# Unrepentant-Atheist/AC-3-ACM-Codec

Hardware: AMD Instinct MI355X
Metric: AC-3 5.1@48kHz frames/sec/GPU (decode+encode); achieved HBM GB/s vs peak (higher is better)
Workload: dtype f32+i32

## Files before the change

ac-3-acm-codec_amd/csrc/decode_mx.hip:

```cpp
#include <stdlib.h>
#include "mant2.h"
#include "xform_core.h"
#include "ac3mi_internal.h"

namespace ac3mi {

constexpr int MX_PLANE = 256 + 16;
constexpr int MX_WAVE = 6 * EX_GROUP * 8;
constexpr int MX_RING = 6 * MX_PLANE * 4;
constexpr int MX_TILE = 3072;
static_assert(MX_RING + M2_LDS_WAVE <= MX_WAVE && MX_TILE + 256 * 6 * 2 <= MX_WAVE && 48 * 8 * 8 <= MX_TILE, "region layout");

struct MantxParams {
    MantParams m;
    const uint8_t *blksw;
    float *delay;
    const int32_t *slot;
    int delay_stride;
    float *pcm;
    int16_t *pcm16;
    int8_t wslot[6];
    const float2 *tw_long, *tw_short;
    const float *window;
    float bias;
// ... 51 lines not shown
    const uint64_t rve = failed ? 0ull : D.rv_exp();
    const uint64_t rvb = failed ? 0ull : D.rv_bap();
    const uint8_t *const rowbase = P.rows + (size_t)fidx * 6 * ROWSET;
    const RowFetch fetch{rowbase, rve, rvb, lane};
    __builtin_assume(B.nf >= 1);
    const int slot0 = seg_slot(0, B.nf, B.chincpl, B.chincpl ? __builtin_ctz(B.chincpl) : 99);
    const uint2 first = fetch(slot0);
    {
        stage_frame_store<384>(frw, fw, P.frame_bytes, tid);
        if (const int own = D.own_bytes()) trim_staged_frame(frw, own, nw, tid, 384);
        if (tid < M2_NDESC) L.dsc[tid] = mant_desc2((uint32_t)tid);
        L.qtab[tid] = q0;
        if (tid < 760 - 384) L.qtab[384 + tid] = q1;
        reinterpret_cast<float2 *>(&L.tw[0][0])[tid] = twv;
        if (tid < 6) L.ready[tid] = 0u;
    }
    __syncthreads();
    MX_LAP(0);

    if (failed) {
        for (int c = 0; c < n_in; c++)
            *reinterpret_cast<float4 *>(planes + c * MX_PLANE + 4 * lane) = make_float4(0.f, 0.f, 0.f, 0.f);
    } else {
        D.ranges(B);
        B.gainv = D.gainv(lane);
        if (B.chincpl && lane < 18) {
            const uint32_t below = D.cplbndstrc() & ((1u << lane) - 1u);
            L.cplbnd[blk][lane] = (uint8_t)(lane - __popc(below));
        }
        const uint32_t fpos = rfl(fposv);
        const bool lfsr_live = fpos != 0xffffffffu;
        const uint32_t i0 = lfsr_live ? (fpos + D.draw_off()) % 65535u : 0u;
        const float *cc = P.cplco + unit * 90;
        mant_block2<MX_PLANE, true>(B, fetch, first, [&](int c, int bnd) { return cc[c * 18 + bnd]; }, L.cplbnd[blk], L.dsc, region + MX_RING, frw,
                              (uint32_t)nw + 2u, L.qtab, reinterpret_cast<const int16_t *>(P.lfsr_seq) + 1 + i0, lfsr_live, planes, D.bitpos(), lane);
    }
    wave_sync();

    MX_LAP(1);
    const int l8 = lane & 7, grp = lane >> 3;
    const bool own = grp < n_in;
    const int o = own ? grp : 0;
    const int fb = o - B.in_lfe;
    const bool sw = fb >= 0 && Q.blksw[unit * nfchans + fb] != 0;
    const size_t sidx = Q.slot ? (size_t)Q.slot[fidx] : (size_t)fidx;
    float *const dptr = Q.delay + sidx * Q.delay_stride + (size_t)o * 128;
    float2 dl[8];
    if (blk == 0) {
#pragma unroll
        for (int j = 0; j < 8; j++) {
            const int i = ((j & 1) ? 15 - l8 : l8) + 16 * (j >> 1);
            dl[j] = *reinterpret_cast<const float2 *>(dptr + 2 * i);
        }
    }
    FirstTail ft;
#pragma unroll
    for (int j = 0; j < 8; j++) ft.f0[j] = ft.f1[j] = ft.t0[j] = ft.t1[j] = 0.f;
    {
        const float *plane = planes + o * MX_PLANE;
        float xa[16], xb[16];
        if (!sw) {
            const float2 *p = reinterpret_cast<const float2 *>(plane) + l8;
            float2 v[16];
#pragma unroll
            for (int n = 0; n < 16; n++) v[n] = p[8 * n];
#pragma unroll
            for (int n = 0; n < 16; n++) {
// ... 31 lines not shown
    if (blk > 0) {
        for (int spin = 0; spin < (1 << 20) && __hip_atomic_load(&L.ready[blk - 1], __ATOMIC_ACQUIRE, __HIP_MEMORY_SCOPE_WORKGROUP) == 0u; spin++)
            __builtin_amdgcn_s_sleep(1);
        const float2 *tl = reinterpret_cast<const float2 *>(L.wave[blk - 1]);
        const int ls = lane < 48 ? lane : l8;
#pragma unroll
        for (int j = 0; j < 8; j++) dl[j] = tl[j * 48 + ls];
    }
    if (blk == 5) {
        for (int spin = 0; spin < (1 << 20) && __hip_atomic_load(&L.ready[0], __ATOMIC_ACQUIRE, __HIP_MEMORY_SCOPE_WORKGROUP) == 0u; spin++)
            __builtin_amdgcn_s_sleep(1);
    }
    if (blk == 5 && own) {
#pragma unroll
        for (int j = 0; j < 8; j++) {
            const int i = ((j & 1) ? 15 - l8 : l8) + 16 * (j >> 1);
            *reinterpret_cast<float2 *>(dptr + 2 * i) = make_float2(ft.t0[j], ft.t1[j]);
        }
    }

    MX_LAP(3);
    int16_t *tile = reinterpret_cast<int16_t *>(region + MX_TILE);
    int wsl = 0;
    if constexpr (FX) {
        uint64_t w = 0;
#pragma unroll
        for (int oo = 0; oo < 6; oo++) w |= (uint64_t)(uint8_t)Q.wslot[oo] << (8 * oo);
        wsl = (int)((uint32_t)(w >> (8 * o)) & 0xffu);
    } else {
#pragma unroll
        for (int oo = 0; oo < 6; oo++) wsl = oo == o ? Q.wslot[oo] : wsl;
    }
    float *oblk = S16 ? nullptr : Q.pcm + (unit * n_in + o) * 256;
#pragma unroll
    for (int j = 0; j < 8; j++) {
        const int i = ((j & 1) ? 15 - l8 : l8) + 16 * (j >> 1);
        const float2 wlo = *reinterpret_cast<const float2 *>(&L.win[2 * i]);
        const float2 whi = *reinterpret_cast<const float2 *>(&L.win[254 - 2 * i]);
        float2 lo, hi;
        window_pair(ft.f0[j], ft.f1[j], dl[j], wlo, whi, Q.bias, lo, hi);
        if (!S16 && own) {
            *reinterpret_cast<float2 *>(oblk + 2 * i) = lo;
            *reinterpret_cast<float2 *>(oblk + 254 - 2 * i) = hi;
        }
        if (S16 && own) {
            const int at = wsl + (int)__umul24((uint32_t)(2 * i), (uint32_t)n_in), top = wsl + (int)__umul24(254u, (uint32_t)n_in) - (at - wsl);
            tile[at] = to_s16(lo.x);
            tile[at + n_in] = to_s16(lo.y);
            tile[top] = to_s16(hi.x);
            tile[top + n_in] = to_s16(hi.y);
        }
    }
    if (S16) {
        wave_sync();
        const int upb = 32 * n_in;
        int16_t *dst = Q.pcm16 + unit * 256 * n_in;
#pragma unroll
        for (int it = 0; it < 3; it++) {
            const int u = it * 64 + lane;
            if (u < upb) *reinterpret_cast<uint4 *>(dst + u * 8) = *reinterpret_cast<const uint4 *>(tile + u * 8);
        }
    }
    MX_LAP(4);
}

template <uint32_t V> struct MantxVariant { static constexpr auto fn = mantx_kernel<(V & V_S16) != 0, (V & V_FX) != 0>; };

hipError_t launch_mantx(const DeviceTables &tab, const DecodeLaunch &L, const MantParams &M, const KernelLaunch &k, hipStream_t stream)
{
    if (!L.fuse) return hipErrorInvalidValue;
    const XformLaunch &X = *L.fuse;
    if (L.frames_per_stream != 1 || X.plan.n_in != X.plan.n_out || M.n_in > 6) return hipErrorInvalidValue;
    MantxParams Q;
    Q.m = M;
    Q.m.coef = nullptr;
    Q.blksw = L.blksw;
    Q.delay = X.delay;
    Q.slot = X.slot;
    Q.delay_stride = X.slot ? X.delay_stride : X.plan.n_out * 128;
// ... 32 lines not shown
```

ac-3-acm-codec_amd/csrc/mant2.h:

```cpp
#pragma once
#include "decode_common.h"

namespace ac3mi {

constexpr int M2_RING = 3 * 128;
constexpr int M2_LDS_WAVE = M2_RING + 256;
constexpr int M2_NDESC = 97;
constexpr int LFSR_EXT = 16384;


struct alignas(16) BlkDesc {
    uint32_t bitpos;
    uint32_t draw_off;
    uint32_t flags;
    uint32_t cplbndstrc;
    uint16_t endmant[5], cplstrt, cplend;
    uint16_t own_bytes;
    uint8_t rv_exp[8], rv_bap[8];
    float gain[5], lfe_gain;
    uint32_t src_snr;
    uint32_t pad1;
};
constexpr uint32_t BLK_FAILED = 1u;
constexpr int BLK_CHINCPL = 8, BLK_DITH = 16, BLK_REMAT = 24;
static_assert(sizeof(BlkDesc) == BLKDESC_BYTES && offsetof(BlkDesc, src_snr) == BLKDESC_SRC_SNR, "what the host sizes and reads (ac3mi_internal.h)");

constexpr int ROWSET = 7 * 512;

static_assert(offsetof(BlkDesc, bitpos) == 0 && offsetof(BlkDesc, draw_off) == 4 && offsetof(BlkDesc, flags) == 8 && offsetof(BlkDesc, cplbndstrc) == 12,
              "lanes 0-3: the first four dwords");
static_assert(offsetof(BlkDesc, cplstrt) == offsetof(BlkDesc, endmant) + 2 * 5 && offsetof(BlkDesc, cplend) == offsetof(BlkDesc, endmant) + 2 * 6 &&
              offsetof(BlkDesc, own_bytes) == offsetof(BlkDesc, endmant) + 2 * 7, "lanes 0-7: eight halfwords from endmant on; 6 = the coupling slot");
static_assert(offsetof(BlkDesc, lfe_gain) == offsetof(BlkDesc, gain) + 4 * 5 && offsetof(BlkDesc, src_snr) == offsetof(BlkDesc, gain) + 4 * 6,
              "lanes 0-6: seven dwords from gain on");
// ... 20 lines not shown
        return (flags & BLK_FAILED) != 0u;
    }
    __device__ __forceinline__ void ranges(MantBlk &B) const
    {
        constexpr size_t E = offsetof(BlkDesc, endmant);
        B.cplstrtmant = (int)s16<offsetof(BlkDesc, cplstrt)>(); B.cplendmant = (int)s16<offsetof(BlkDesc, cplend)>();
        B.ends = (uint64_t)((s16<E>() & 0xffu) | ((s16<E + 2>() & 0xffu) << 8) | ((s16<E + 4>() & 0xffu) << 16) | ((s16<E + 6>() & 0xffu) << 24)) |
                 ((uint64_t)(s16<E + 8>() & 0xffu) << 32);
    }
    __device__ __forceinline__ float gainv(int lane) const
    {
        constexpr size_t G = offsetof(BlkDesc, gain);
        return __uint_as_float(lane == 0 ? u32<G>() : lane == 1 ? u32<G + 4>() : lane == 2 ? u32<G + 8>() : lane == 3 ? u32<G + 12>()
                             : lane == 4 ? u32<G + 16>() : u32<offsetof(BlkDesc, lfe_gain)>());
    }
    __device__ __forceinline__ int own_bytes() const { return (int)s16<offsetof(BlkDesc, own_bytes)>(); }
    __device__ __forceinline__ uint32_t cplbndstrc() const { return s32<offsetof(BlkDesc, cplbndstrc)>(); }
    __device__ __forceinline__ uint32_t bitpos() const { return s32<offsetof(BlkDesc, bitpos)>(); }
    __device__ __forceinline__ uint32_t draw_off() const { return s32<offsetof(BlkDesc, draw_off)>(); }
    __device__ __forceinline__ uint64_t rv_exp() const { return (uint64_t)s32<offsetof(BlkDesc, rv_exp)>() | ((uint64_t)s32<offsetof(BlkDesc, rv_exp) + 4>() << 32); }
    __device__ __forceinline__ uint64_t rv_bap() const { return (uint64_t)s32<offsetof(BlkDesc, rv_bap)>() | ((uint64_t)s32<offsetof(BlkDesc, rv_bap) + 4>() << 32); }
};

struct RowFetch {
    const uint8_t *const &rowbase;
    const uint64_t &rve, &rvb;
    const int &lane;
    __device__ __forceinline__ uint2 operator()(int slot) const
    {
        const uint8_t *er = rowbase + (size_t)((rve >> (8 * slot)) & 7u) * ROWSET + slot * 512;
        const uint8_t *br = rowbase + (size_t)((rvb >> (8 * slot)) & 7u) * ROWSET + slot * 512 + 256;
        if (slot == 5) return lane < 7 ? make_uint2(br[lane], er[lane]) : make_uint2(1u, 0u);
        return make_uint2(reinterpret_cast<const uint32_t *>(br)[lane], reinterpret_cast<const uint32_t *>(er)[lane]);
    }
};

__host__ __device__ inline uint4 mant_desc2(uint32_t b)
{
    const uint32_t k1 = b >> 5, nbp = b >= 32 ? 0u : b == 1 ? 0u : b;
    const uint32_t inc = k1 == 1 ? 1u << 20 : k1 == 2 ? 1u << 10 : k1 == 3 ? 1u : 0u;
    const uint32_t obits = k1 == 1 ? 5u : k1 ? 7u : 0u, per = k1 == 3 ? 2u : k1 ? 3u : 0u, sh = 30u - 10u * k1;
    const uint32_t recip = k1 == 3 ? 1024u : k1 ? 683u : 0u;
    const uint32_t qbase = k1 == 1 ? 0u : k1 == 2 ? 96u : k1 == 3 ? 480u : nbp == 3 ? 736u : nbp == 4 ? 744u : 0u;
    const uint32_t coded = (k1 || nbp == 3 || nbp == 4) ? 1u : 0u, zero = b == 0 ? 1u : 0u;
    const uint32_t ring = k1 ? 128u * (k1 - 1u) : 0u;
    return make_uint4(inc, nbp | (obits << 8) | (per << 16) | (sh << 24), recip | (qbase << 16), ring | (zero << 16) | (coded << 24));
}

struct MantParams {
    const uint8_t *frames;
    const BlkDesc *desc;
    const uint8_t *rows;
    const float *cplco;
    const uint32_t *frame_pos;
    float *coef;
    const uint16_t *lfsr_seq;
    const DecTables *tab;
    unsigned n_frames;
    int frame_stride, frame_bytes;
    int acmod, lfeon, n_in, nfchans;
};

struct Seg2 {
    uint32_t bit;
    uint32_t phase;
    uint32_t draw;
// ... 24 lines not shown
    uint32_t nb[NB], nbsum = 0, ndsum = 0, slot[NB];
#pragma unroll
    for (int j = 0; j < NB; j++) {
        const uint32_t x = __builtin_amdgcn_ubfe(run, R.dy[j] >> 24, 10);
        run += inc[j];
        const uint32_t q = (x * (R.dz[j] & 0xffffu)) >> 11;
        const uint32_t mem = x - q * ((R.dy[j] >> 16) & 0xffu);
        const uint32_t ob = mem == 0u ? (R.dy[j] >> 8) & 0xffu : 0u;
        nb[j] = (R.dy[j] & 0xffu) + ob;
        nbsum += nb[j];
        ndsum += ((R.dw[j] >> 16) & 0xffu) * (uint32_t)mult;
        const uint32_t rslot = (R.dw[j] & 0xffffu) + (q & 127u);
        R.rs[j] = rslot | (mem << 16);
        slot[j] = ob != 0u ? rslot : (uint32_t)(M2_RING + 4 * lane);
    }
    const uint32_t bl = nbsum | (ndsum << 16);
    const uint32_t bin_ = wave_incl_scan_u32(bl);
    const uint32_t gtot = wave_last(gin), btot = wave_last(bin_);
    R.cd = S.draw + (bin_ >> 16) - ndsum;
    const uint32_t off = S.bit + (bin_ & 0xffffu) - nbsum;
    uint32_t wi = off >> 5;
    wi = wi < frw_last ? wi : frw_last;
    const uint32_t d0 = frw[wi], d1 = frw[wi + 1], d2 = frw[wi + 2];
    const uint32_t k = off & 31u;
    uint64_t win = ((((uint64_t)d0 << 32) | d1) << k) | (uint64_t)((d2 >> 1) >> (31u - k));
#pragma unroll
    for (int j = 0; j < NB; j++) {
        R.raw[j] = ((uint32_t)(win >> 32) >> 1) >> (31u - nb[j]);
        win <<= nb[j];
        ring[slot[j]] = (uint8_t)R.raw[j];
    }
    S.bit += btot & 0xffffu;
    S.draw += btot >> 16;
    {
        const uint32_t x3 = ((S.phase >> 20) & 1023u) + ((gtot >> 20) & 1023u), x5 = ((S.phase >> 10) & 1023u) + ((gtot >> 10) & 1023u),
                       x11 = (S.phase & 1023u) + (gtot & 1023u);
        const uint32_t q3 = (x3 * 683u) >> 11, q5 = (x5 * 683u) >> 11, q11 = x11 >> 1;
        S.phase = (((q3 & 127u) * 3u + (x3 - 3u * q3)) << 20) | (((q5 & 127u) * 3u + (x5 - 3u * q5)) << 10) | ((q11 & 127u) * 2u + (x11 & 1u));
    }
}

template <int NB>
__device__ __forceinline__ void seg2_values(const Bins2<NB> &R, const uint8_t *ring, const float *qtab, float *q)
{
    uint32_t code[NB];
#pragma unroll
    for (int j = 0; j < NB; j++) code[j] = ring[R.rs[j] & 0xffffu];
#pragma unroll
    for (int j = 0; j < NB; j++) { asm volatile("" : "+v"(code[j])); code[j] &= 0xffu; }
    float tv[NB];
#pragma unroll
    for (int j = 0; j < NB; j++) {
        const uint32_t per = (R.dy[j] >> 16) & 0xffu;
        const uint32_t sel = per ? code[j] * per + (R.rs[j] >> 16) : R.raw[j];
        tv[j] = qtab[(R.dw[j] >> 24) ? (R.dz[j] >> 16) + sel : 0u];
    }
#pragma unroll
    for (int j = 0; j < NB; j++) {
        const uint32_t nbp = R.dy[j] & 0xffu;
        const float pv = (float)(((int32_t)(R.raw[j] << ((32u - nbp) & 31u))) >> 16);
        q[j] = (R.dw[j] >> 24) ? tv[j] : pv;
    }
}

__device__ __forceinline__ float dither2(const int16_t *seq, uint32_t i) { return (float)((3 * (int)seq[i]) >> 2); }

template <int PS = 256, bool PK = false, class Fetch, class Cplco>
__device__ __forceinline__ void mant_block2(const MantBlk &B, Fetch fetch, uint2 first, Cplco cplco_of, const uint8_t *cplbnd, const uint4 *dsc, uint8_t *ring,
                                            const uint32_t *frw, uint32_t frw_last, const float *qtab, const int16_t *seq1, bool lfsr_live,
                                            float *cblk, uint32_t bitpos, int lane)
{
    const int nf = B.nf;
    const int ncpl_dith = __popc(B.chincpl & B.dithmask);
    const int em0 = PK ? (int)((uint32_t)B.ends & 0xffu) : B.endmant[0], em1 = PK ? (int)(((uint32_t)B.ends >> 8) & 0xffu) : B.endmant[1];
    const int remat_end = em0 < em1 ? em0 : em1;
    const bool remat_late = B.acmod == 2 && B.rematflg != 0 && B.chincpl != 0 && remat_end > B.cplstrtmant;
    const int cplfirst = B.chincpl ? __builtin_ctz(B.chincpl) : 99;
    const int nseg = nf + (B.chincpl ? 1 : 0) + (B.lfeon ? 1 : 0);
    Seg2 S;
    S.bit = bitpos;
    S.phase = 0;
    S.draw = 0;
    uint2 nxt = first;
    for (int k = 0; k < nseg; k++) {
        const int slot = seg_slot(k, nf, B.chincpl, cplfirst);
        const uint2 cur = nxt;
        if (k + 1 < nseg) nxt = fetch(seg_slot(k + 1, nf, B.chincpl, cplfirst));
        if (slot == 5) {
            Bins2<1> R;
            seg2_first<1>(lane < 7 ? cur.x & 0xffu : 1u, dsc, ring, frw, frw_last, 0, S, R, lane);
            wave_sync();
            float q;
            seg2_values<1>(R, ring, qtab, &q);
            const float lfe_gain = PK ? __builtin_bit_cast(float, __builtin_amdgcn_readlane(__builtin_bit_cast(int, B.gainv), 5)) : B.lfe_gain;
            const float v = q * (sf_of((int)(cur.y & 0xffu)) * lfe_gain);
            const float z = 0.f * (sf_of(0) * lfe_gain);
            if (lane < 8) cblk[lane] = lane < 7 ? v : z;
            if (lane >= 2) *reinterpret_cast<float4 *>(cblk + 4 * lane) = make_float4(z, z, z, z);
            continue;
        }
        int start = 0, end, draws;
        float g = 0.f;
        if (slot < 5) {
            if (PK) {
                end = (int)((uint32_t)(B.ends >> (8 * slot)) & 0xffu);
                g = __builtin_bit_cast(float, __builtin_amdgcn_readlane(__builtin_bit_cast(int, B.gainv), slot));
            } else {
                end = slot == 0 ? B.endmant[0] : slot == 1 ? B.endmant[1] : slot == 2 ? B.endmant[2] : slot == 3 ? B.endmant[3] : B.endmant[4];
                g = slot == 0 ? B.gain[0] : slot == 1 ? B.gain[1] : slot == 2 ? B.gain[2] : slot == 3 ? B.gain[3] : B.gain[4];
            }
            draws = (B.dithmask >> slot) & 1;
        } else {
            start = B.cplstrtmant;
            end = B.cplendmant;
            draws = ncpl_dith;
        }
        uint32_t bytes4;
        {
            int lo = start - 4 * lane, hi = end - 4 * lane;
            lo = lo < 0 ? 0 : lo > 4 ? 4 : lo;
            hi = hi < 0 ? 0 : hi > 4 ? 4 : hi;
            const uint32_t below_hi = (uint32_t)((1ull << (8 * hi)) - 1ull), below_lo = (uint32_t)((1ull << (8 * lo)) - 1ull);
            const uint32_t m = below_hi & ~below_lo;
            bytes4 = (cur.x & m) | (0x01010101u & ~m);
        }
        Bins2<4> R;
        seg2_first<4>(bytes4, dsc, ring, frw, frw_last, draws, S, R, lane);
        wave_sync();
        if (slot < 5) {
            float out[4], qv[4];
            seg2_values<4>(R, ring, qtab, qv);
            const bool dith = draws != 0 && lfsr_live;
            const uint32_t z0 = (R.dw[0] >> 16) & 0xffu, z1 = (R.dw[1] >> 16) & 0xffu, z2 = (R.dw[2] >> 16) & 0xffu, z3 = (R.dw[3] >> 16) & 0xffu;
            if (dith && __any((z0 | z1 | z2 | z3) != 0u)) {
                const int16_t *sp = seq1 + R.cd;
                const float d0 = dither2(sp, 0), d1 = dither2(sp, z0), d2 = dither2(sp, z0 + z1), d3 = dither2(sp, z0 + z1 + z2);
                qv[0] = z0 ? d0 : qv[0]; qv[1] = z1 ? d1 : qv[1]; qv[2] = z2 ? d2 : qv[2]; qv[3] = z3 ? d3 : qv[3];
            }
#pragma unroll
            for (int j = 0; j < 4; j++) {
                const int e = (int)((cur.y >> (8 * j)) & 0xffu);
                out[j] = qv[j] * (sf_of(e) * g);
            }
            float *plane = cblk + (slot + B.in_lfe) * PS;
            if (slot == 1 && B.acmod == 2 && B.rematflg != 0 && !remat_late) {
                float4 a4 = *reinterpret_cast<const float4 *>(plane - PS + 4 * lane);
                float a[4] = {a4.x, a4.y, a4.z, a4.w};
#pragma unroll
                for (int j = 0; j < 4; j++) {
                    const int bin = 4 * lane + j;
                    const int band = bin < 25 ? 0 : bin < 37 ? 1 : bin < 61 ? 2 : 3;
                    if (bin >= 13 && (bin < remat_end || (bin == 13 && remat_end <= 13)) && ((B.rematflg >> band) & 1)) {
                        const float x = a[j], v = out[j];
                        a[j] = x + v;
                        out[j] = x - v;
                    }
                }
                *reinterpret_cast<float4 *>(plane - PS + 4 * lane) = make_float4(a[0], a[1], a[2], a[3]);
            }
            if ((B.chincpl >> slot) & 1) {
#pragma unroll
                for (int j = 0; j < 4; j++) {
                    const int bin = 4 * lane + j;
                    if (bin < end || bin < B.cplstrtmant || bin >= B.cplendmant) plane[bin] = bin >= B.cplendmant ? 0.f : out[j];
                }
            } else {
                *reinterpret_cast<float4 *>(plane + 4 * lane) = make_float4(out[0], out[1], out[2], out[3]);
            }
        } else {
            uint32_t cd = R.cd;
// ... 43 lines not shown
```

ac-3-acm-codec_amd/csrc/encode.hip:

```cpp
#include "ac3mi_internal.h"
#include "wave_ops.h"
#include "spec_tables.h"
#include "enc_mant.h"
#include "enc_syntax.h"
#include "enc_exp.h"
#include "snr_window.h"
#include "crc_lanes.h"
#include "mdct_rule.h"

#include <type_traits>

namespace ac3mi {

__device__ __forceinline__ int ilog2u(unsigned v) { return v ? 31 - __builtin_clz(v) : 0; }

__device__ __forceinline__ int wave_sum(int v) { return (int)wave_sum_u32((uint32_t)v); }


struct PackParams {
    const int32_t *mdct;
    const uint8_t *eexp;
    const int16_t *emask;
    const uint8_t *strat;
    const int32_t *ebits;
    const int8_t *shift;
    int32_t *csnr_state;
    const int32_t *slot;
    int32_t *snr;
    uint32_t *memo;
    uint8_t *frames;
    const EncTables *tab;
    uint8_t *tap_eexp;
    uint8_t *tap_bap;
    uint8_t *tap_strat;
    int32_t *tap_snr;
    int32_t *tap_curve;
    int n_streams, frames_per_stream, frame_stride;
    int nch, nfbw, lfe, acmod, fscod, halfrate, bsid, frmsizecod, frame_words;
    int nbc;
    int chbwcod;
    const uint16_t *crc_rows;
    int crc_c, crc_n1;
    int frw;
    int marker;
    const uint32_t *hint;
    int hint_stride;
    const uint8_t *bsw;
    const uint8_t *remat;
    CplWs cpl;
    int cpl_begf;
    int cpl_endf;
    const uint8_t *drc;
    uint32_t bsi;
    const uint32_t *bsi_words;
    const uint8_t *dyn;
    const uint16_t *compr;
};

__device__ __forceinline__ uint32_t pack_bsi(const PackParams &P, size_t fidx)
{
    return P.bsi_words ? bsi_sanitise((uint32_t)__builtin_amdgcn_readfirstlane((int)P.bsi_words[fidx])) : P.bsi;
}

__device__ __forceinline__ bool drc_sends(const uint8_t *code, int b) { return b == 0 || code[b] != code[b - 1]; }
__device__ __forceinline__ bool dyn_sends(const uint8_t *code, int b, int p) { return code[2 * b + p] != (b ? code[2 * b - 2 + p] : 0); }
__device__ __forceinline__ uint32_t compr_word(const PackParams &P, size_t fidx, int p)
{
    return P.compr ? (uint32_t)__builtin_amdgcn_readfirstlane((int)P.compr[fidx * 2 + p]) & 0x1ffu : 0u;
}

template <bool MD, bool DW>
__device__ __forceinline__ uint32_t pack_dynrng(const PackParams &P, size_t fidx, int b, int p)
{
    if constexpr (DW) if (P.dyn) return dyn_sends(P.dyn + fidx * 12, b, p) ? 0x100u | P.dyn[fidx * 12 + 2 * b + p] : 0u;
    if constexpr (MD) if (P.drc && drc_sends(P.drc + fidx * 6, b)) return 0x100u | P.drc[fidx * 6 + b];
    return 0u;
}

struct MaskTabs {
// ... 243 lines not shown
    const int b = lane;
    const int cur = b < bndend ? bndpsd[b] : 0;
    const int nxt = (b + 1 < bndend && !(is_lfe && b == 6)) ? bndpsd[b + 1] : 0;
    const bool skip = (is_lfe && b == 6) || b >= 22 || b >= bndend;
    const bool reset = !skip && b < 20 && cur + 256 == nxt;
    const int dec = skip || reset ? 0 : b >= 20 ? 2 : (cur > nxt ? 1 : 0);
    const int D = (int)wave_incl_scan_u32((uint32_t)dec);
    const int rix = wave_incl_scan_max(reset ? b : NEG);
    const int Dr = __shfl(D, rix < 0 ? 0 : rix, 64);
    int lowcomp = 0;
    if (rix >= 0) { lowcomp = (rix < 7 ? 384 : 320) - 64 * (D - Dr); lowcomp = lowcomp < 0 ? 0 : lowcomp; }

    const bool stop = b >= 2 && b < 7 && b < bndend && !(is_lfe && b == 6) && cur <= nxt;
    const unsigned long long sm = __ballot(stop);
    const int begin = sm ? __builtin_ctzll(sm) + 1 : 7;
    const bool live = b >= begin - 1 && b < bndend;
    int fast, slow;
    mask_leaks(cur, live, b, sdecay, fdecay, sgain, fgain, fast, slow);
    int excite;
    if (b < begin) excite = (int16_t)(cur - fgain - lowcomp);
    else if (b < 22) { const int v = fast - lowcomp; excite = (int16_t)(slow > v ? slow : v); }
    else excite = (int16_t)(fast > slow ? fast : slow);
    mask_store(T, bndpsd, b, b < bndend, excite, cur, dbknee, halfrate);
}


struct ExpParams {
    uint8_t *eexp;
    int16_t *emask;
    uint8_t *strat;
    int32_t *ebits;
    const EncTables *tab;
    int nch, lfe, fscod, halfrate, nbc;
};

struct ExpLDS {
    uint8_t E[6][256];
    int16_t mask[6][50];
    MaskTabs t;
    uint8_t strat[8];
};

template <bool KEEP = false, int XS = 0, bool FX = false>
__device__ void exp_stage(const ExpParams &P, ExpLDS &L, size_t fidx, int ch, int lane)
{
    const int nch = FX ? 6 : P.nch;
    const bool is_lfe = (FX || P.lfe) && ch == nch - 1;
    const int n = is_lfe ? 7 : FX ? 223 : P.nbc;
    uint32_t raw[6];
#pragma unroll
    for (int b = 0; b < 6; b++) raw[b] = *reinterpret_cast<const uint32_t *>(&L.E[b][4 * lane]);
    uint32_t below = 0;
#pragma unroll
    for (int c = 0; c < 4; c++) below |= (4 * lane + c < n ? 0xffu : 0u) << (8 * c);

    int st[6];
    st[0] = 1;
    if constexpr (KEEP) {
#pragma unroll
        for (int b = 0; b < 6; b++) st[b] = (int)P.strat[(fidx * 6 + b) * nch + ch];
    } else if constexpr (XS != 0) {
        const uint32_t x = xs_choose<false>(L.E, nullptr, below, n, 0, 0, is_lfe ? 0 : XS == 1 ? 8 : 2, is_lfe, lane);
#pragma unroll
        for (int b = 0; b < 6; b++) st[b] = (int)((x >> (4 * b)) & 15u);
    } else {
        const uint32_t d1 = __builtin_amdgcn_sad_u8(raw[1], raw[0], 0u), d2 = __builtin_amdgcn_sad_u8(raw[2], raw[1], 0u);
// ... 62 lines not shown
            const int nb = slot < 5 ? 1 : slot < 7 ? 2 : slot == 7 ? 4 : slot == 8 ? 2 : 7;
            const int lw = slot < 5 ? 3 : slot < 7 ? 2 : slot < 9 ? 1 : 0;
            const bool rowon = lane < 60 && ((starts >> r) & 1u);
            const int rr = rowon ? r : 0;
            const int start = L.t.band_start[fb];
            int end1 = L.t.band_start[fb + nb];
            end1 = end1 < n ? end1 : n;
            const int len = rowon ? end1 - start : 0;
            const uint32_t *q = reinterpret_cast<const uint32_t *>(&L.E[rr][start & ~3]);
            uint32_t dw[7], ab[6];
#pragma unroll
            for (int i = 0; i < 7; i++) dw[i] = q[i];
#pragma unroll
            for (int i = 0; i < 6; i++) ab[i] = __builtin_amdgcn_alignbyte(dw[i + 1], dw[i], (uint32_t)start & 3u);
            int16_t *mrow = &L.mask[rr][fb];
            const bool r3 = lw == 0, r6 = lw <= 1, r12 = lw <= 2;
            int v = 3072 - ((int)(ab[0] & 0xffu) << 7);
#pragma unroll
            for (int j = 1; j < 24; j++) {
                const int pj = 3072 - ((int)((ab[j >> 2] >> (8 * (j & 3))) & 0xffu) << 7);
                int t = (int)(__builtin_amdgcn_sad_u16((uint32_t)v, (uint32_t)pj, 0u) >> 1);
                t = t > 255 ? 255 : t;
                int nv = (v > pj ? v : pj) + (int)L.t.latab[t];
                if (j % 3 == 0) {
                    const bool ends = j % 12 == 0 ? r12 : j % 6 == 0 ? r6 : r3;
                    if (ends && j < len) mrow[((j / 3) >> lw) - 1] = (int16_t)v;
                    nv = ends ? pj : nv;
                }
                v = j < len ? nv : v;
            }
            if (len > 0) mrow[((((uint32_t)(len - 1)) * 0xaaabu) >> 17) >> lw] = (int16_t)v;
        }
        wave_sync();
        const int sdecaycod = 2, fdecaycod = 1, fgaincod = 4;
        constexpr int sgaincod = 1, dbkneecod = 2;
        const int sdecay = enc_sdecay(sdecaycod) >> P.halfrate, fdecay = enc_fdecay(fdecaycod) >> P.halfrate;
        const int sgain = enc_sgain(sgaincod), dbknee = enc_dbknee(dbkneecod), fgain = enc_fgain(fgaincod);
        const int bndend = L.t.band_of_bin[n - 1] + 1;
        for (uint32_t m = starts; m; m &= m - 1)
            mask_row_wave(L.t, L.mask[__builtin_ctz(m)], bndend, is_lfe, sdecay, fdecay, sgain, dbknee, fgain, P.halfrate, lane);
    }
    wave_sync();

    static_assert(enc_floor(4) == 0x1f0 && enc_sgain(1) == 0x4d8 && enc_dbknee(2) == 0x900, "ENC/ac3tab.h:151-161");
    {
        typedef short short2v __attribute__((ext_vector_type(2)));
        const int half = lane >= 25 ? 1 : 0, k2 = lane - 25 * half;
        int src[6];
        src[0] = 0;
#pragma unroll
        for (int b = 1; b < 6; b++) src[b] = ((starts >> b) & 1u) ? b : src[b - 1];
#pragma unroll
        for (int it = 0; it < 3; it++) {
            const int b = 2 * it + half, sr = half ? src[2 * it + 1] : src[2 * it];
            if (lane < 50) {
                short2v v = *reinterpret_cast<const short2v *>(&L.mask[sr][2 * k2]);
                v -= (short2v){(short)enc_floor(4), (short)enc_floor(4)};
                *reinterpret_cast<short2v *>(P.emask + ((fidx * 6 + b) * nch + ch) * 50 + 2 * k2) = v;
            }
        }
    }
    if (lane < 6) P.strat[(fidx * 6 + lane) * nch + ch] = L.strat[lane];
    if (lane == 0) P.ebits[fidx * nch + ch] = exp_bits;
}


// ... 808 lines not shown
        const uint8_t *cex = cplf ? P.cpl.eexp + fidx * 6 * 256 : ex;
        bool loaded = false;
        auto load_frame = [&]() {
            loaded = true;
            if constexpr (!WIN) {
                const uint32_t *gm = reinterpret_cast<const uint32_t *>(P.emask + fidx * 6 * nch * 50);
                uint32_t mv[15];
#pragma unroll
                for (int j = 0; j < 15; j++) {
                    const int i = lane + 64 * j;
                    mv[j] = i < 6 * nch * 25 ? gm[i] : 0;
                }
#pragma unroll
                for (int j = 0; j < 15; j++) {
                    const int i = lane + 64 * j;
                    if (i < 6 * nch * 25) reinterpret_cast<uint32_t *>(&L.mask[0][0])[i] = mv[j];
                }
            }
            if (lane < 6 * nch) { const int b = lane / nch, ch = lane - b * nch; L.strat[b][ch] = P.strat[fidx * 6 * nch + lane]; }
            frame_bits = wave_sum(lane < nch ? P.ebits[fidx * nch + lane] : 0);
            wave_sync();
            {
                const int b6 = lane / 6, c6 = lane - 6 * b6;
                row_set = __ballot(lane < 36 && c6 < nch && L.strat[lane < 36 ? b6 : 0][c6] != 0);
                const int c8 = lane >> 3, b8 = lane & 7;
                run_starts = __ballot(b8 < 6 && c8 < nch && L.strat[b8 < 6 ? b8 : 0][c8 < 6 ? c8 : 0] != 0);
                if (lane < 36 && ((row_set >> lane) & 1)) {
                    const uint32_t later = (uint32_t)((run_starts >> (8 * c6)) & 0x3f) | 0x40u;
                    const int b1 = __builtin_ctz(later >> (b6 + 1)) + b6 + 1;
                    const uint32_t cover = ((1u << b1) - 1u) & ~((1u << b6) - 1u);
                    uint32_t d = (uint32_t)((b6 * nch + c6) * 256) | ((lfe && c6 == nch - 1) ? 1u << 14 : 0u) | (cover << 16) | ((uint32_t)(b6 * nch + c6) << 24);
                    if constexpr (CPL) d |= cplf && c6 < nfbw ? 1u << 22 : 0u;
                    L.rowdesc[__builtin_popcountll(row_set & ((1ull << lane) - 1ull))] = d;
                }
            }
            {
                frame_bits += syn_priced_fixed(acmod, lfe, nfbw, nch);
                uint64_t fbw_rows = 0;
                for (int b = 0; b < 6; b++) fbw_rows |= ((1ull << nfbw) - 1) << (6 * b);
                frame_bits += 8 * __builtin_popcountll(row_set & fbw_rows);
                if constexpr (DRC) if (!DW || P.drc) {
                    const uint8_t *code = P.drc + fidx * 6;
                    for (int b = 0; b < 6; b++) frame_bits += drc_sends(code, b) ? (acmod == 0 ? 16 : 8) : 0;
                }
                if constexpr (DW) {
                    const int np = acmod == 0 ? 2 : 1;
                    if (P.dyn) {
                        const uint8_t *code = P.dyn + fidx * 12;
                        for (int b = 0; b < 6; b++)
                            for (int p = 0; p < np; p++) frame_bits += dyn_sends(code, b, p) ? 8 : 0;
                    }
                    for (int p = 0; p < np; p++) frame_bits += (compr_word(P, fidx, p) & 0x100u) ? 8 : 0;
                }
                if (!FX && P.remat)
                    for (int b = 1; b < 6; b++) frame_bits += (P.remat[fidx * 6 + b] & 0x10) ? 4 : 0;
                if (CPL && cplf) {
                    frame_bits += syn_priced_cpl(acmod, nfbw, cpl_nb);
                    frame_bits += __builtin_amdgcn_readfirstlane(P.cpl.ebits[fidx]) - 6 * __builtin_popcountll(row_set & fbw_rows);
                    if (P.remat) {
                        const int nrem = syn_cpl_nrem(P.cpl_begf);
                        for (int b = 1; b < 6; b++) frame_bits -= (P.remat[fidx * 6 + b] & 0x10) ? 4 - nrem : 0;
                    }
                }
            }
            if constexpr (CPL) if (cplf) {
                if constexpr (!WIN) {
// ... 1069 lines not shown

hipError_t launch_encode(const DeviceTables &tab, const EncodeLaunch &E, hipStream_t stream)
{
    if (E.n_streams <= 0 || E.frames_per_stream <= 0) return hipSuccess;
    const EncConfig &c = E.cfg;
    const EncChoice R = enc_choice(E);
    if (R.err) return hipErrorInvalidValue;
    hipError_t e;
    if (R.drc && (e = launch_drc(E, stream)) != hipSuccess) return e;
    MdctParams M;
    M.pcm = E.pcm;
    M.last = E.last;
    M.mdct = E.ws_mdct;
    M.full_rows = E.mdct_full_rows ? 1 : 0;
    M.expo = E.ws_expo;
    M.shift = E.ws_shift;
    M.tab = tab.enc;
    M.n_streams = E.n_streams;
    M.frames = E.frames_per_stream;
    M.nch = c.nch;
    for (int i = 0; i < 8; i++) M.chmap[i] = E.chmap[i];
    M.slot = E.slot;
    M.store_history = !R.history;
    M.x.eexp = E.ws_eexp;
    M.x.emask = E.ws_emask;
    M.x.strat = E.ws_strat;
    M.x.ebits = E.ws_ebits;
    M.x.tab = tab.enc;
    M.x.nch = c.nch;
    M.x.lfe = c.lfe;
    M.x.fscod = c.fscod;
    M.x.halfrate = c.halfrate;
    M.x.nbc = R.nbc;
    M.bsw = E.ws_bsw;
    M.remat = R.remat ? E.ws_remat : nullptr;
    if (R.stage[ES_PRE].family != K_NONE) {
        MdctParams M0 = M;
        M0.mdct = E.ws_cpl.prow;
        M0.shift = E.ws_cpl.pshift;
        M0.expo = nullptr;
        M0.full_rows = 1;
        M0.store_history = 0;
        M0.remat = nullptr;
        M0.x.eexp = E.ws_cpl.peexp;
        M0.x.emask = E.ws_cpl.pemask;
        M0.x.strat = E.ws_cpl.pstrat;
        M0.x.ebits = E.ws_cpl.pebits;
        if ((e = launch_stage<ENC_MDCT_VARIANTS, MdctVariant>(R.stage[ES_PRE], E, 0, stream, M0)) != hipSuccess) return e;
    }
    if ((e = launch_stage<ENC_MDCT_VARIANTS, MdctVariant>(R.stage[ES_MDCT], E, 0, stream, M)) != hipSuccess) return e;
    {
        MdctParams ML = M;
        ML.remat = nullptr;
        if ((e = launch_stage<ENC_MDCT_VARIANTS, MdctVariant>(R.stage[ES_LFEROW], E, 0, stream, ML)) != hipSuccess) return e;
    }
    if (R.cpl) {
        CplParams C;
        C.mdct = E.ws_mdct;
        C.shift = E.ws_shift;
        C.bsw = E.ws_bsw;
        C.remat = M.remat;
        C.mdct_out = E.ws_mdct;
        C.shift_out = E.ws_shift;
        C.w = E.ws_cpl;
        C.x = M.x;
        C.x.nbc = 37 + 12 * E.cpl_begf;
// ... 15 lines not shown
    P.csnr_state = E.csnr;
    P.slot = E.slot;
    P.frames = E.frames;
    P.tab = tab.enc;
    P.tap_eexp = E.tap_eexp;
    P.tap_bap = E.tap_bap;
    P.tap_strat = E.tap_strat;
    P.tap_snr = E.tap_snr;
    P.tap_curve = E.tap_curve;
    P.n_streams = E.n_streams;
    P.frames_per_stream = E.frames_per_stream;
    P.frame_stride = E.frame_stride;
    P.nch = c.nch;
    P.nfbw = c.nfbw;
    P.lfe = c.lfe;
    P.acmod = c.acmod;
    P.fscod = c.fscod;
    P.halfrate = c.halfrate;
    P.bsid = c.bsid;
    P.frmsizecod = c.frmsizecod;
    P.frame_words = c.frame_words;
    P.nbc = R.nbc;
    P.chbwcod = E.chbwcod;
    const int fs = c.frame_words;
    if (!E.crc_rows) return hipErrorInvalidValue;
    const CrcSplit split = crcl_split(fs);
    P.crc_rows = E.crc_rows;
    P.crc_c = split.C;
    P.crc_n1 = split.n1;
    P.snr = E.ws_snr;
    P.memo = R.memo ? E.ws_memo : nullptr;
    P.hint = E.search_hint;
    P.hint_stride = E.search_hint_stride;
    P.bsw = E.ws_bsw;
    P.remat = M.remat;
    P.cpl = R.cpl ? E.ws_cpl : CplWs{};
    P.cpl_begf = R.cpl ? E.cpl_begf : 0;
    P.cpl_endf = R.cpl_endf;
    P.drc = R.drc ? E.ws_drc_code : nullptr;
    P.bsi = E.bsi;
    P.bsi_words = E.bsi_words;
    P.dyn = E.dyn_codes;
    P.compr = E.compr_words;
#ifndef ENC_FR_HEADROOM
#define ENC_FR_HEADROOM 256
#endif
    P.frw = ((2 * fs + ENC_FR_HEADROOM + 15) / 16) * 4;
    P.marker = getenv("AC3MI_ENC_MARKER") ? atoi(getenv("AC3MI_ENC_MARKER")) : 128;
    static const int lds_pad = getenv("AC3MI_ENC_LDS_PAD") ? atoi(getenv("AC3MI_ENC_LDS_PAD")) : 0;
    const size_t fr_lds = (size_t)P.frw * 4 + lds_pad;
    if ((e = launch_stage<ENC_SEARCH_VARIANTS, SearchVariant>(R.stage[ES_TABULATE], E, 0, stream, P)) != hipSuccess) return e;
    if ((e = launch_stage<ENC_SEARCH_VARIANTS, SearchVariant>(R.stage[ES_SEARCH], E, 0, stream, P)) != hipSuccess) return e;
    e = R.packb ? launch_stage<ENC_PACKB_VARIANTS, PackbVariant>(R.stage[ES_PACK], E, fr_lds, stream, P)
                : launch_stage<ENC_PACKF_VARIANTS, PackfVariant>(R.stage[ES_PACK], E, fr_lds, stream, P);
    if (e != hipSuccess) return e;
    return R.history ? launch_enc_history(E, stream) : hipSuccess;
}

__global__ void enc_history_kernel(const int16_t *pcm, int16_t *last, int n_streams, int frames, int nch, const uint8_t c0,
                                   const uint8_t c1, const uint8_t c2, const uint8_t c3, const uint8_t c4, const uint8_t c5,
                                   const int32_t *slot)
{
    const uint8_t chmap[6] = {c0, c1, c2, c3, c4, c5};
    const int idx = blockIdx.x * blockDim.x + threadIdx.x;
    if (idx >= n_streams * nch * 256) return;
    const int j = idx & 255, ch = (idx >> 8) % nch, s = (idx >> 8) / nch;
// ... 45 lines not shown
```

Baseline: 9.985 million.

## Merge LFE mantissa segment into last fbw channel segment and simplify tile addressing

When the LFE channel is on and the last full-bandwidth segment ends early enough (at most 224 bins), the 7 LFE mantissas ride in the upper lanes (56+) of that segment's wave pass. This removes one whole segment iteration, with its scan and wave_sync, per block. The change also swaps the grouped-mantissa phase update for a cheaper modular form and hoists the S16 tile index math out of the unroll loop. The ride path relies on the LFE bins being decoded in bitstream order right after the host channel, which only holds when coupling does not sit between them, so the new eligibility checks and phase arithmetic could introduce correctness issues.

Measured after the change: 9.960 million. No clear change (-0.3%).

```diff
diff --git a/ac-3-acm-codec_amd/csrc/decode_mx.hip b/ac-3-acm-codec_amd/csrc/decode_mx.hip
--- a/ac-3-acm-codec_amd/csrc/decode_mx.hip
+++ b/ac-3-acm-codec_amd/csrc/decode_mx.hip
@@ -107,7 +107,7 @@
         const bool lfsr_live = fpos != 0xffffffffu;
         const uint32_t i0 = lfsr_live ? (fpos + D.draw_off()) % 65535u : 0u;
         const float *cc = P.cplco + unit * 90;
-        mant_block2<MX_PLANE, true>(B, fetch, first, [&](int c, int bnd) { return cc[c * 18 + bnd]; }, L.cplbnd[blk], L.dsc, region + MX_RING, frw,
+        mant_block2<MX_PLANE, true, true>(B, fetch, first, [&](int c, int bnd) { return cc[c * 18 + bnd]; }, L.cplbnd[blk], L.dsc, region + MX_RING, frw,
                               (uint32_t)nw + 2u, L.qtab, reinterpret_cast<const int16_t *>(P.lfsr_seq) + 1 + i0, lfsr_live, planes, D.bitpos(), lane);
     }
     wave_sync();
@@ -205,6 +205,8 @@
         for (int oo = 0; oo < 6; oo++) wsl = oo == o ? Q.wslot[oo] : wsl;
     }
     float *oblk = S16 ? nullptr : Q.pcm + (unit * n_in + o) * 256;
+    const int at0 = wsl + (int)__umul24((uint32_t)(2 * l8), (uint32_t)n_in), at1 = wsl + (int)__umul24((uint32_t)(2 * (15 - l8)), (uint32_t)n_in);
+    const int top0 = 2 * wsl + (int)__umul24(254u, (uint32_t)n_in) - at0, top1 = 2 * wsl + (int)__umul24(254u, (uint32_t)n_in) - at1;
 #pragma unroll
     for (int j = 0; j < 8; j++) {
         const int i = ((j & 1) ? 15 - l8 : l8) + 16 * (j >> 1);
@@ -217,7 +219,8 @@
             *reinterpret_cast<float2 *>(oblk + 254 - 2 * i) = hi;
         }
         if (S16 && own) {
-            const int at = wsl + (int)__umul24((uint32_t)(2 * i), (uint32_t)n_in), top = wsl + (int)__umul24(254u, (uint32_t)n_in) - (at - wsl);
+            const int step = (j >> 1) * 32 * n_in;
+            const int at = ((j & 1) ? at1 : at0) + step, top = ((j & 1) ? top1 : top0) - step;
             tile[at] = to_s16(lo.x);
             tile[at + n_in] = to_s16(lo.y);
             tile[top] = to_s16(hi.x);
diff --git a/ac-3-acm-codec_amd/csrc/mant2.h b/ac-3-acm-codec_amd/csrc/mant2.h
--- a/ac-3-acm-codec_amd/csrc/mant2.h
+++ b/ac-3-acm-codec_amd/csrc/mant2.h
@@ -1,5 +1,6 @@
 #pragma once
 #include "decode_common.h"
+#include "mant_ride.h"
 
 namespace ac3mi {
 
@@ -86,6 +87,13 @@
         const uint8_t *br = rowbase + (size_t)((rvb >> (8 * slot)) & 7u) * ROWSET + slot * 512 + 256;
         if (slot == 5) return lane < 7 ? make_uint2(br[lane], er[lane]) : make_uint2(1u, 0u);
         return make_uint2(reinterpret_cast<const uint32_t *>(br)[lane], reinterpret_cast<const uint32_t *>(er)[lane]);
+    }
+    __device__ __forceinline__ uint32_t ride() const
+    {
+        const uint8_t *er = rowbase + (size_t)((rve >> 40) & 7u) * ROWSET + 5 * 512;
+        const uint8_t *br = rowbase + (size_t)((rvb >> 40) & 7u) * ROWSET + 5 * 512 + 256;
+        const int k = mant_ride_bin(lane);
+        return k >= 0 ? mant_ride_byte(br[k]) | ((uint32_t)er[k] << 8) : 1u;
     }
 };
 
@@ -176,12 +184,7 @@
     }
     S.bit += btot & 0xffffu;
     S.draw += btot >> 16;
-    {
-        const uint32_t x3 = ((S.phase >> 20) & 1023u) + ((gtot >> 20) & 1023u), x5 = ((S.phase >> 10) & 1023u) + ((gtot >> 10) & 1023u),
-                       x11 = (S.phase & 1023u) + (gtot & 1023u);
-        const uint32_t q3 = (x3 * 683u) >> 11, q5 = (x5 * 683u) >> 11, q11 = x11 >> 1;
-        S.phase = (((q3 & 127u) * 3u + (x3 - 3u * q3)) << 20) | (((q5 & 127u) * 3u + (x5 - 3u * q5)) << 10) | ((q11 & 127u) * 2u + (x11 & 1u));
-    }
+    S.phase = seg2_phase_next(S.phase, gtot);
 }
 
 template <int NB>
@@ -209,7 +212,7 @@
 
 __device__ __forceinline__ float dither2(const int16_t *seq, uint32_t i) { return (float)((3 * (int)seq[i]) >> 2); }
 
-template <int PS = 256, bool PK = false, class Fetch, class Cplco>
+template <int PS = 256, bool PK = false, bool RIDE = false, class Fetch, class Cplco>
 __device__ __forceinline__ void mant_block2(const MantBlk &B, Fetch fetch, uint2 first, Cplco cplco_of, const uint8_t *cplbnd, const uint4 *dsc, uint8_t *ring,
                                             const uint32_t *frw, uint32_t frw_last, const float *qtab, const int16_t *seq1, bool lfsr_live,
                                             float *cblk, uint32_t bitpos, int lane)
@@ -220,16 +223,25 @@
     const int remat_end = em0 < em1 ? em0 : em1;
     const bool remat_late = B.acmod == 2 && B.rematflg != 0 && B.chincpl != 0 && remat_end > B.cplstrtmant;
     const int cplfirst = B.chincpl ? __builtin_ctz(B.chincpl) : 99;
-    const int nseg = nf + (B.chincpl ? 1 : 0) + (B.lfeon ? 1 : 0);
+    const int host_end = PK ? (int)((uint32_t)(B.ends >> (8 * (nf - 1))) & 0xffu)
+                            : nf == 1 ? B.endmant[0] : nf == 2 ? B.endmant[1] : nf == 3 ? B.endmant[2] : nf == 4 ? B.endmant[3] : B.endmant[4];
+    const bool rides = RIDE && mant_lfe_rides(B.lfeon, nf, B.chincpl, host_end);
+    const int nseg = nf + (B.chincpl ? 1 : 0) + (B.lfeon && !rides ? 1 : 0);
     Seg2 S;
     S.bit = bitpos;
     S.phase = 0;
     S.draw = 0;
     uint2 nxt = first;
+    uint32_t rid = 1u;
+    if (rides && nseg == 1) rid = fetch.ride();
     for (int k = 0; k < nseg; k++) {
         const int slot = seg_slot(k, nf, B.chincpl, cplfirst);
         const uint2 cur = nxt;
-        if (k + 1 < nseg) nxt = fetch(seg_slot(k + 1, nf, B.chincpl, cplfirst));
+        if (k + 1 < nseg) {
+            nxt = fetch(seg_slot(k + 1, nf, B.chincpl, cplfirst));
+            if (rides && k + 2 == nseg) rid = fetch.ride();
+        }
+        const bool merged = rides && k + 1 == nseg;
         if (slot == 5) {
             Bins2<1> R;
             seg2_first<1>(lane < 7 ? cur.x & 0xffu : 1u, dsc, ring, frw, frw_last, 0, S, R, lane);
@@ -268,6 +280,7 @@
             const uint32_t m = below_hi & ~below_lo;
             bytes4 = (cur.x & m) | (0x01010101u & ~m);
         }
+        if (merged) bytes4 = mant_ride_bytes(lane, bytes4, rid & 0xffu);
         Bins2<4> R;
         seg2_first<4>(bytes4, dsc, ring, frw, frw_last, draws, S, R, lane);
         wave_sync();
@@ -280,6 +293,14 @@
                 const int16_t *sp = seq1 + R.cd;
                 const float d0 = dither2(sp, 0), d1 = dither2(sp, z0), d2 = dither2(sp, z0 + z1), d3 = dither2(sp, z0 + z1 + z2);
                 qv[0] = z0 ? d0 : qv[0]; qv[1] = z1 ? d1 : qv[1]; qv[2] = z2 ? d2 : qv[2]; qv[3] = z3 ? d3 : qv[3];
+            }
+            if (merged) {
+                const float lfe_gain = PK ? __builtin_bit_cast(float, __builtin_amdgcn_readlane(__builtin_bit_cast(int, B.gainv), 5)) : B.lfe_gain;
+                const float v = qv[0] * (sf_of((int)(rid >> 8)) * lfe_gain);
+                const float z = 0.f * (sf_of(0) * lfe_gain);
+                if (lane >= RIDE_LANE0) cblk[lane - RIDE_LANE0] = v;
+                if (lane >= 2) *reinterpret_cast<float4 *>(cblk + 4 * lane) = make_float4(z, z, z, z);
+                qv[0] = lane >= RIDE_LANE0 ? 0.f : qv[0];
             }
 #pragma unroll
             for (int j = 0; j < 4; j++) {
diff --git a/ac-3-acm-codec_amd/csrc/mant_ride.h b/ac-3-acm-codec_amd/csrc/mant_ride.h
--- /dev/null
+++ b/ac-3-acm-codec_amd/csrc/mant_ride.h
@@ -0,0 +1,38 @@
+#pragma once
+#include <stdint.h>
+
+#ifndef __HIPCC__
+#ifndef __host__
+#define __host__
+#endif
+#ifndef __device__
+#define __device__
+#endif
+#endif
+
+namespace ac3mi {
+
+constexpr int RIDE_LANE0 = 56, RIDE_BINS = 7, RIDE_MAX_END = 4 * RIDE_LANE0;
+
+__host__ __device__ inline bool mant_lfe_rides(int lfeon, int nf, int chincpl, int host_end)
+{
+    const bool cpl_between = chincpl != 0 && (chincpl & ((1 << (nf - 1)) - 1)) == 0;
+    return lfeon != 0 && !cpl_between && host_end <= RIDE_MAX_END;
+}
+
+__host__ __device__ inline int mant_ride_bin(int lane) { return lane >= RIDE_LANE0 && lane < RIDE_LANE0 + RIDE_BINS ? lane - RIDE_LANE0 : -1; }
+
+__host__ __device__ inline uint32_t mant_ride_byte(uint32_t lfe_byte) { return lfe_byte ? lfe_byte : 1u; }
+
+__host__ __device__ inline int mant_bin_draws(uint32_t b, int draws) { return b == 0u ? draws : 0; }
+
+__host__ __device__ inline uint32_t mant_ride_bytes(int lane, uint32_t host4, uint32_t ride_byte) { return lane >= RIDE_LANE0 ? 0x01010100u | ride_byte : host4; }
+
+__host__ __device__ inline uint32_t seg2_phase_next(uint32_t phase, uint32_t total)
+{
+    const uint32_t s = phase + total;
+    const uint32_t x3 = (s >> 20) & 1023u, x5 = (s >> 10) & 1023u;
+    return ((x3 >= 384u ? x3 - 384u : x3) << 20) | ((x5 >= 384u ? x5 - 384u : x5) << 10) | (s & 255u);
+}
+
+}
```

## Move masking curve computation from exponent stage into search kernel per-lane rows

Applied to the files above, without the earlier changes.

For the fixed-layout variant, the exponent stage now writes the banded PSD rows, strategy and exponent bits, then returns early without running the wave-serial masking walk. The search kernel instead loads all 36 rows into LDS, and each lane computes one block/channel masking curve with a new scalar mask_rule routine before writing the curves back to global memory. This swaps a per-row wave-cooperative computation for lane-parallel serial walks. The cost is extra global traffic, an LDS round-trip in the search kernel and higher register pressure.

After: 9.977 million before, 10.07 million after (median of 6 runs). No clear change (+0.9%).

```diff
diff --git a/ac-3-acm-codec_amd/csrc/encode.hip b/ac-3-acm-codec_amd/csrc/encode.hip
--- a/ac-3-acm-codec_amd/csrc/encode.hip
+++ b/ac-3-acm-codec_amd/csrc/encode.hip
@@ -7,6 +7,7 @@
 #include "snr_window.h"
 #include "crc_lanes.h"
 #include "mdct_rule.h"
+#include "mask_rule.h"
 
 #include <type_traits>
 
@@ -45,6 +46,7 @@
     int marker;
     const uint32_t *hint;
     int hint_stride;
+    int psd_rows;
     const uint8_t *bsw;
     const uint8_t *remat;
     CplWs cpl;
@@ -354,6 +356,7 @@
     int32_t *ebits;
     const EncTables *tab;
     int nch, lfe, fscod, halfrate, nbc;
+    int psd_rows;
 };
 
 struct ExpLDS {
@@ -482,6 +485,18 @@
             if (len > 0) mrow[((((uint32_t)(len - 1)) * 0xaaabu) >> 17) >> lw] = (int16_t)v;
         }
         wave_sync();
+        if constexpr (FX) if (P.psd_rows) {
+            const int half = lane >= 25 ? 1 : 0, k2 = lane - 25 * half;
+#pragma unroll
+            for (int it = 0; it < 3; it++) {
+                const int b = 2 * it + half;
+                if (lane < 50 && ((starts >> b) & 1u))
+                    reinterpret_cast<uint32_t *>(P.emask + ((fidx * 6 + b) * nch + ch) * 50)[k2] = reinterpret_cast<const uint32_t *>(&L.mask[b][0])[k2];
+            }
+            if (lane < 6) P.strat[(fidx * 6 + lane) * nch + ch] = L.strat[lane];
+            if (lane == 0) P.ebits[fidx * nch + ch] = exp_bits;
+            return;
+        }
         const int sdecaycod = 2, fdecaycod = 1, fgaincod = 4;
         constexpr int sgaincod = 1, dbkneecod = 2;
         const int sdecay = enc_sdecay(sdecaycod) >> P.halfrate, fdecay = enc_fdecay(fdecaycod) >> P.halfrate;
@@ -1356,6 +1371,35 @@
                     uint32_t d = (uint32_t)((b6 * nch + c6) * 256) | ((lfe && c6 == nch - 1) ? 1u << 14 : 0u) | (cover << 16) | ((uint32_t)(b6 * nch + c6) << 24);
                     if constexpr (CPL) d |= cplf && c6 < nfbw ? 1u << 22 : 0u;
                     L.rowdesc[__builtin_popcountll(row_set & ((1ull << lane) - 1ull))] = d;
+                }
+                if constexpr (FX) if (P.psd_rows) {
+                    static_assert(offsetof(SearchWindowBufs, hist) == sizeof(SearchWindowBufs::scan) &&
+                                  sizeof(SearchWindowBufs::scan) + sizeof(SearchWindowBufs::hist) >= 36 * 25 * 4, "36 rows of 25 dwords");
+                    uint32_t *rows = &L.scan[0];
+                    uint32_t *gm = reinterpret_cast<uint32_t *>(const_cast<int16_t *>(P.emask)) + fidx * 900;
+                    uint32_t mv[15];
+#pragma unroll
+                    for (int j = 0; j < 15; j++) mv[j] = gm[j < 14 || lane < 4 ? lane + 64 * j : 896];
+                    const int hv = (int)P.tab->hth[(lane < 50 ? lane : 49) >> P.halfrate][P.fscod];
+#pragma unroll
+                    for (int j = 0; j < 15; j++) if (j < 14 || lane < 4) rows[lane + 64 * j] = mv[j];
+                    wave_sync();
+                    const int rl = lane < 36 ? lane : 35, rb = lane < 36 ? b6 : 5, rc = lane < 36 ? c6 : 5;
+                    const uint32_t sent = (uint32_t)(run_starts >> (8 * rc)) & ((2u << rb) - 1u);
+                    const int src = (31 - __builtin_clz(sent | 1u)) * 6 + rc;
+                    const MaskCodes mc = {enc_sdecay(2) >> P.halfrate, enc_fdecay(1) >> P.halfrate, enc_sgain(1), enc_dbknee(2), enc_fgain(4), enc_floor(4)};
+                    uint32_t curve[25];
+                    mask_rule_row(reinterpret_cast<const int16_t *>(rows + 25 * src), 1, rc == 5 ? 7 : L.band_of_bin[222] + 1, rc == 5, mc,
+                                  [&](int b) { return __builtin_amdgcn_readlane(hv, b); }, curve);
+                    wave_sync();
+#pragma unroll
+                    for (int k = 0; k < 25; k++) rows[25 * rl + k] = curve[k];
+                    wave_sync();
+#pragma unroll
+                    for (int j = 0; j < 15; j++) if (j < 14 || lane < 4) gm[lane + 64 * j] = rows[lane + 64 * j];
+                    asm volatile("s_waitcnt vmcnt(0)" ::: "memory");
+                    if (lane == 0) L.scan[3] = 0;
+                    wave_sync();
                 }
             }
             {
@@ -2491,6 +2535,9 @@
     M.x.fscod = c.fscod;
     M.x.halfrate = c.halfrate;
     M.x.nbc = R.nbc;
+    const bool mask_rows = R.stage[ES_MDCT].variant == V_FX && R.stage[ES_SEARCH].variant == (1u | V_FX) &&
+                           !(getenv("AC3MI_ENC_MASK_ROWS") && atoi(getenv("AC3MI_ENC_MASK_ROWS")) == 0);
+    M.x.psd_rows = mask_rows ? 1 : 0;
     M.bsw = E.ws_bsw;
     M.remat = R.remat ? E.ws_remat : nullptr;
     if (R.stage[ES_PRE].family != K_NONE) {
@@ -2572,6 +2619,7 @@
     P.memo = R.memo ? E.ws_memo : nullptr;
     P.hint = E.search_hint;
     P.hint_stride = E.search_hint_stride;
+    P.psd_rows = M.x.psd_rows;
     P.bsw = E.ws_bsw;
     P.remat = M.remat;
     P.cpl = R.cpl ? E.ws_cpl : CplWs{};
diff --git a/ac-3-acm-codec_amd/csrc/mask_rule.h b/ac-3-acm-codec_amd/csrc/mask_rule.h
--- /dev/null
+++ b/ac-3-acm-codec_amd/csrc/mask_rule.h
@@ -0,0 +1,76 @@
+#pragma once
+#include <stdint.h>
+
+#ifndef __HIPCC__
+#ifndef __host__
+#define __host__
+#endif
+#ifndef __device__
+#define __device__
+#endif
+#endif
+
+namespace ac3mi {
+
+struct MaskCodes {
+    int sdecay, fdecay, sgain, dbknee, fgain, floor;
+};
+
+template <class Psd, class Hth>
+__host__ __device__ inline void mask_rule_walk(Psd psd_of, int bndend, bool is_lfe, const MaskCodes &c, Hth hth_of, uint32_t *out)
+{
+    int lowcomp = 0, fast = 0, slow = 0;
+    bool begun = false;
+    uint32_t lo16 = 0;
+    int cur = psd_of(0);
+#if defined(__HIP_DEVICE_COMPILE__)
+#pragma unroll
+#endif
+    for (int b = 0; b < 50; b++) {
+        int nxt = 0;
+        if (b + 1 < 50) { const int stored = psd_of(b + 1); nxt = b + 1 < bndend ? stored : 0; }
+        const bool lfe6 = b == 6 && is_lfe;
+        if (b < 20) {
+            const int down = lowcomp - 64;
+            int lc = cur > nxt ? (down < 0 ? 0 : down) : lowcomp;
+            lc = cur + 256 == nxt ? (b < 7 ? 384 : 320) : lc;
+            lowcomp = lfe6 ? lowcomp : lc;
+        } else if (b < 22) {
+            const int down = lowcomp - 128;
+            lowcomp = down < 0 ? 0 : down;
+        }
+        const int fg = cur - c.fgain, sg = cur - c.sgain;
+        int excite;
+        if (b < 2) {
+            excite = (int16_t)(fg - lowcomp);
+        } else {
+            const bool leak = b >= 7 || begun;
+            const int fl = fast - c.fdecay, sl = slow - c.sdecay;
+            fast = leak && fl > fg ? fl : fg;
+            slow = leak && sl > sg ? sl : sg;
+            if (b < 22) {
+                const int v = fast - lowcomp;
+                excite = (int16_t)(leak && slow > v ? slow : v);
+            } else {
+                excite = (int16_t)(fast > slow ? fast : slow);
+            }
+            if (b < 7) begun = begun || (!lfe6 && cur <= nxt);
+        }
+        const int t = c.dbknee - cur;
+        excite += (t > 0 ? t : 0) >> 2;
+        const int h = hth_of(b);
+        const int m = (b < bndend ? (excite > h ? excite : h) : 0) - c.floor;
+        if (b & 1) out[b >> 1] = lo16 | (uint32_t)m << 16;
+        else lo16 = (uint32_t)m & 0xffffu;
+        cur = nxt;
+    }
+}
+
+template <class Hth>
+__host__ __device__ inline void mask_rule_row(const int16_t *psd, int stride, int bndend, bool is_lfe, const MaskCodes &c,
+                                              Hth hth_of, uint32_t *out)
+{
+    mask_rule_walk([=](int b) { return (int)psd[b * stride]; }, bndend, is_lfe, c, hth_of, out);
+}
+
+}
```
